# malak29/video-text-detection-system

Hardware: AMD Instinct MI355X
Metric: frames/sec (detect+recognize) @720p, 1/2/4/8 MI355X; box IoU vs CPU ref (higher is better)
Workload: dtype f16

## Files before the change

video-text-detection-system_amd/build_native.py:

```python
import glob
import os
import subprocess
import sys

HERE = os.path.dirname(os.path.abspath(__file__))
CSRC = os.path.join(HERE, "csrc")
OUT_DIR = os.path.join(HERE, "vtd_amd", "_lib")
VARIANT = os.environ.get("VTD_LIB_VARIANT", "")
EXTRA = os.environ.get("VTD_EXTRA_HIPCC_FLAGS", "").split()
if EXTRA and not VARIANT:
    raise SystemExit("VTD_EXTRA_HIPCC_FLAGS needs VTD_LIB_VARIANT=<tag>: the product library is only ever built with the default flags")
OUT = os.path.join(OUT_DIR, f"libvtd_hip_{VARIANT}.so" if VARIANT else "libvtd_hip.so")
OBJ_DIR = os.path.join(HERE, f"build_{VARIANT}" if VARIANT else "build")

COMMON = ["--offload-arch=gfx950", "-O3", "-fPIC", "-std=c++17", "-Wall", "-Wno-unused-function", "-mllvm", "-amdgpu-mfma-vgpr-form",
          "-I" + CSRC] + EXTRA
PER_FILE = {"postprocess.hip": ["-ffp-contract=off"], "adamw.hip": ["-ffp-contract=off"]}


def sources():
    src = glob.glob(os.path.join(CSRC, "*.hip")) + glob.glob(os.path.join(CSRC, "*.cpp"))
    if "-DVTD_EXPERIMENTAL_CANDIDATES" in EXTRA:
        src += glob.glob(os.path.join(CSRC, "experimental", "*.hip"))
    return sorted(src)


def build(force=False, verbose=False):
    os.makedirs(OUT_DIR, exist_ok=True)
    os.makedirs(OBJ_DIR, exist_ok=True)
    headers = (glob.glob(os.path.join(CSRC, "*.h")) + glob.glob(os.path.join(CSRC, "*.inc")) +
               glob.glob(os.path.join(HERE, "..", "include", "*.h")))
    newest_hdr = max(os.path.getmtime(h) for h in headers)
# ... 44 lines not shown
```

video-text-detection-system_amd/csrc/conv_halo.hip:

```cpp
#include <cstdio>
#include <cstdlib>
#include "vtd_common.h"

namespace {

struct HaloParams {
    const half_t* in;
    const half_t* wgt;
    const float* bias;
    const half_t* res;
    half_t* out;
    int n, h, w, cin, cout;
    int in_hp, in_wp, in_ring, out_hp, out_wp, out_ring, res_hp, res_wp, res_ring;
    int tiles_x, tiles_y, tiles_n, relu;
    unsigned long long* stamps;
    int dbg;
};

template <int N>
__device__ __forceinline__ void hl_wait_vmcnt() {
    asm volatile("s_waitcnt vmcnt(%0)" ::"n"(N) : "memory");
}

template <int BN, int TW>
__global__ __launch_bounds__((BN / 64) * 256) void conv_halo_kernel(const HaloParams p) {
    constexpr int WN = BN / 64, NW = 4 * WN, NT = NW * 64, TH = 256 / TW;
    constexpr int HWD = TW + 2, HROWS = (TH + 2) * HWD, HPIECES = (HROWS + 7) / 8, HBYTES = HPIECES * 1024;
    constexpr int HPW = (HPIECES + NW - 1) / NW;
    constexpr int HPS = (HPW + 7) / 8;
    constexpr int BSTAGE = BN * 128, BPW = BN / 8 / NW;
    constexpr int EPI_ROW = BN * 4 + 16;
// ... 499 lines not shown
template <int TW, bool RELU, bool RES>
__global__ __launch_bounds__(512, 1) void conv3x3_c64_duo_kernel(const HaloParams p) {
    constexpr int TH = 256 / TW, HWD = TW + 2, HROWS = (TH + 2) * HWD, HPIECES = (HROWS + 7) / 8, HBYTES = HPIECES * 1024;
    constexpr int HPW = (HPIECES + 3) / 4;
    constexpr int WBYTES = 9 * 64 * 128;
    extern __shared__ __attribute__((aligned(16))) char smem[];
    char* const wl = smem;
    char* const hbuf = smem + WBYTES;

    const int tid = threadIdx.x, lane = tid & 63;
    const int wv = __builtin_amdgcn_readfirstlane(tid >> 6);
    const int g = wv >> 2, w = wv & 3;
    const int lrow = lane >> 3, fr = lane & 15, fq = lane >> 4;
    const int tiles_per_img = p.tiles_x * p.tiles_y, total = p.n * tiles_per_img;

#pragma unroll
    for (int k = 0; k < 9; ++k) {
        const int piece = wv + 8 * k, tap = piece >> 3, row = (piece & 7) * 8 + lrow;
        const int c_log = (lane & 7) ^ ((row >> 1) & 7);
        const int cout = 16 * ((row & 15) >> 2) + 4 * (row >> 4) + (row & 3);
        __builtin_amdgcn_global_load_lds((const VTD_AS1 void*)(p.wgt + cout * 576 + tap * 64 + c_log * 8),
                                         (VTD_AS3 void*)(wl + piece * 1024), 16, 0, 0);
    }
    float* const bias_lds = (float*)(smem + WBYTES + 2 * HBYTES + 1024);
    if (tid < 64) bias_lds[tid] = p.bias[tid];

    auto tile_coords = [&](int t, int& img, int& y0, int& x0) {
        img = t / tiles_per_img;
        const int r = t - img * tiles_per_img, ty = r / p.tiles_x;
        y0 = ty * TH;
        x0 = (r - ty * p.tiles_x) * TW;
    };
    auto issue_halo = [&](int t) {
        int img, y0, x0;
        tile_coords(t, img, y0, x0);
        const half_t* base = p.in + ((int64_t)(img * p.in_hp + y0 - 1 + p.in_ring) * p.in_wp + x0 - 1 + p.in_ring) * 64;
#pragma unroll
        for (int k = 0; k < HPW; ++k) {
            const int piece = w + 4 * k;
            int row = piece * 8 + lrow;
            row = row < HROWS ? row : HROWS - 1;
            const int hy = row / HWD, hx = row - hy * HWD;
            const int hrel = (hy * p.in_wp + hx) * 64 + ((lane & 7) ^ (hx & 6)) * 8;
            const int hdst = piece < HPIECES ? WBYTES + g * HBYTES + piece * 1024 : WBYTES + 2 * HBYTES;
            __builtin_amdgcn_global_load_lds((const VTD_AS1 void*)(base + hrel), (VTD_AS3 void*)(smem + hdst), 16, 0, 0);
        }
    };
    auto px_row = [&](int j) { return (w * 64 + j * 16 + fr) / TW; };
    auto px_col = [&](int j) { return (w * 64 + j * 16 + fr) % TW; };
    const int a_lane_off = (px_row(0) * HWD + px_col(0)) * 128;
    const int b_lane_off = fr * 128;
    const int bswz = (fr >> 1) & 7;
    const char* const hb = hbuf + g * HBYTES;

    const int nq = (total - (int)blockIdx.x + (int)gridDim.x - 1) / (int)gridDim.x;
    const int nmine = (nq - g + 1) >> 1;
    const int phases = 2 * ((nq + 1) >> 1) > 2 * (nq >> 1) + 1 ? 2 * ((nq + 1) >> 1) : 2 * (nq >> 1) + 1;
#ifdef VTD_CONV_EXPERIMENT
    auto block_of = [&](int i) { return p.dbg == 1 ? (int)blockIdx.x : (int)blockIdx.x + (2 * i + g) * (int)gridDim.x; };
#else
    auto block_of = [&](int i) { return (int)blockIdx.x + (2 * i + g) * (int)gridDim.x; };
#endif

    if (nmine > 0) issue_halo(block_of(0));
    hl_wait_vmcnt<0>();
    asm volatile("s_waitcnt lgkmcnt(0)" ::: "memory");
    __builtin_amdgcn_s_barrier();

    floatx4 acc[4][4];
    half8 rv[4][2];
    for (int phase = 0; phase < phases; ++phase) {
        if ((phase & 1) == g) {
            const int i = (phase - g) >> 1;
            if (i < nmine) {
                if (RES) {
                    int img, y0, x0;
                    tile_coords(block_of(i), img, y0, x0);
                    const half_t* rbase = p.res + ((int64_t)(img * p.res_hp + y0 + p.res_ring) * p.res_wp + x0 + p.res_ring) * 64;
#pragma unroll
                    for (int j = 0; j < 4; ++j) {
                        const int rrel = (px_row(j) * p.res_wp + px_col(j)) * 64 + fq * 16;
                        rv[j][0] = *(const half8*)(rbase + rrel);
                        rv[j][1] = *(const half8*)(rbase + rrel + 8);
                    }
                }
#pragma unroll
                for (int a = 0; a < 4; ++a)
#pragma unroll
                    for (int j = 0; j < 4; ++j) acc[a][j] = *(const floatx4*)(bias_lds + fq * 16 + a * 4);
                auto load_frags = [&](int hs, half8 (&af)[4], half8 (&bf)[4]) {
                    const int tap = hs >> 1, kk = hs & 1;
                    const int tapoff = (tap / 3) * HWD + (tap % 3), dx = tap % 3;
// ... 14 lines not shown
#pragma unroll
                        for (int j = 0; j < 4; ++j)
                            acc[a][j] = __builtin_amdgcn_mfma_f32_16x16x32_f16(fb[hs & 1][a], fa[hs & 1][j], acc[a][j], 0, 0, 0);
                    if (hs + 1 < 18) {
                        __builtin_amdgcn_sched_group_barrier(0x100, 8, 0);
                        __builtin_amdgcn_sched_group_barrier(0x008, 16, 0);
                    }
                    __builtin_amdgcn_sched_barrier(0);
                    if (hs + 1 < 18) {
#pragma unroll
                        for (int j = 0; j < 4; ++j) asm volatile("" ::"v"(fa[(hs + 1) & 1][j]));
#pragma unroll
                        for (int a = 0; a < 4; ++a) asm volatile("" ::"v"(fb[(hs + 1) & 1][a]));
                    }
                }
            }
        } else {
            const int i = (phase - g - 1) >> 1;
            if (phase - g - 1 >= 0 && i < nmine) {
                if (i + 1 < nmine) issue_halo(block_of(i + 1));
                int img, y0, x0;
                tile_coords(block_of(i), img, y0, x0);
                half_t* obase = p.out + ((int64_t)(img * p.out_hp + y0 + p.out_ring) * p.out_wp + x0 + p.out_ring) * 64;
#pragma unroll
                for (int j = 0; j < 4; ++j)
#pragma unroll
                    for (int h = 0; h < 2; ++h) {
                        half8 hv;
#pragma unroll
                        for (int k = 0; k < 8; ++k) {
                            float v = acc[2 * h + (k >> 2)][j][k & 3];
                            if (RES) v += (float)rv[j][h][k];
                            hv[k] = (half_t)(RELU ? fmaxf(v, 0.f) : v);
                        }
                        *(half8*)(obase + (px_row(j) * p.out_wp + px_col(j)) * 64 + fq * 16 + h * 8) = hv;
                    }
            }
            hl_wait_vmcnt<0>();
        }
        __builtin_amdgcn_s_barrier();
    }
    hl_wait_vmcnt<0>();
}

template <int TW, bool RELU, bool RES>
int c64_launch(const HaloParams& p, hipStream_t stream) {
    constexpr int TH = 256 / TW, HROWS = (TH + 2) * (TW + 2), HBYTES = (HROWS + 7) / 8 * 1024;
    constexpr int lds = 9 * 64 * 128 + 2 * HBYTES + 1024 + 256;
    static_assert(lds <= 160 * 1024, "LDS budget");
    if (p.h % TH || p.w % TW) return -2205;
    static bool attr_done = false;
    if (!attr_done) {
        hipError_t e = hipFuncSetAttribute((const void*)conv3x3_c64_persistent_kernel<TW, RELU, RES>,
                                           hipFuncAttributeMaxDynamicSharedMemorySize, lds);
        if (e != hipSuccess) return -(int)e;
        attr_done = true;
    }
    const int total = p.n * p.tiles_y * p.tiles_x;
    const int grid = total < 256 ? total : 256;
    static const bool want_stamps = [] { const char* e = getenv("VTD_HALO_STAMPS"); return e && e[0] == '1'; }();
    if (want_stamps) {
        HaloParams q = p;
        unsigned long long* dev = nullptr;
// ... 2 lines not shown
        hipLaunchKernelGGL((conv3x3_c64_persistent_kernel<TW, RELU, RES>), dim3(grid), dim3(256), lds, stream, q);
        (void)hipStreamSynchronize(stream);
        unsigned long long* h = (unsigned long long*)malloc((size_t)grid * 32);
        (void)hipMemcpy(h, dev, (size_t)grid * 32, hipMemcpyDeviceToHost);
        double a = 0, b = 0, c = 0;
        for (int i = 0; i < grid; ++i) { a += (double)h[4 * i + 1]; b += (double)(h[4 * i + 2] - h[4 * i + 1]); c += (double)(h[4 * i + 3] - h[4 * i + 2]); }
        const double blocks = (double)total / grid;
        fprintf(stderr, "[c64 stamps] res=%d blocks/WG %.1f: per block ticks: issue+wait %.1f  K-loop %.1f  epilogue %.1f\n", (int)RES, blocks,
                a / grid / blocks, b / grid / blocks, c / grid / blocks);
        free(h);
        (void)hipFree(dev);
        return 0;
    }
    const char* duo_env = getenv("VTD_C64_DUO");
    const bool duo = !(duo_env && duo_env[0] == '0');
#ifdef VTD_CONV_EXPERIMENT
    if (duo) {
        HaloParams q = p;
        const char* d = getenv("VTD_C64_DEBUG");
        q.dbg = d ? atoi(d) : 0;
        hipError_t e = hipFuncSetAttribute((const void*)conv3x3_c64_duo_kernel<TW, RELU, RES>, hipFuncAttributeMaxDynamicSharedMemorySize, lds);
        if (e != hipSuccess) return -(int)e;
        hipLaunchKernelGGL((conv3x3_c64_duo_kernel<TW, RELU, RES>), dim3(grid), dim3(512), lds, stream, q);
        return -(int)hipGetLastError();
    }
#endif
    if (duo) {
        static bool attr_duo = false;
        if (!attr_duo) {
            hipError_t e = hipFuncSetAttribute((const void*)conv3x3_c64_duo_kernel<TW, RELU, RES>, hipFuncAttributeMaxDynamicSharedMemorySize, lds);
            if (e != hipSuccess) return -(int)e;
            attr_duo = true;
        }
        hipLaunchKernelGGL((conv3x3_c64_duo_kernel<TW, RELU, RES>), dim3(grid), dim3(512), lds, stream, p);
        return -(int)hipGetLastError();
    }
    hipLaunchKernelGGL((conv3x3_c64_persistent_kernel<TW, RELU, RES>), dim3(grid), dim3(256), lds, stream, p);
    return -(int)hipGetLastError();
}

template <int TW>
int c64_dispatch(const HaloParams& p, hipStream_t stream) {
    if (p.relu) return p.res ? c64_launch<TW, true, true>(p, stream) : c64_launch<TW, true, false>(p, stream);
    return p.res ? c64_launch<TW, false, true>(p, stream) : c64_launch<TW, false, false>(p, stream);
}

template <int BN, int TW>
int halo_launch(const HaloParams& p, hipStream_t stream) {
    constexpr int TH = 256 / TW, HROWS = (TH + 2) * (TW + 2), HBYTES = (HROWS + 7) / 8 * 1024;
// ... 46 lines not shown
    if (c.in_y0 < 0 || c.in_x0 != c.in_y0 || c.ho <= 0 || c.wo <= 0 || c.M % (c.ho * c.wo)) return false;
    const int h = c.ho, w = c.wo;
    auto eff = [&](int th, int tw) { return (double)h * w / ((double)((h + th - 1) / th * th) * ((w + tw - 1) / tw * tw)); };
    const double e16 = eff(16, 16), e32 = eff(8, 32);
    const int tw = e16 >= e32 ? 16 : 32;
    if ((tw == 16 ? e16 : e32) < 0.85) return false;
    *tw_out = tw;
    *bn_out = (c.cout % 128 == 0) ? 128 : 64;
    return true;
}

bool vtd_conv_halo_c64_supported(const ConvParams& c, int tw) {
    return c.in_c == 64 && c.cout == 64 && c.wo % tw == 0 && c.ho % (256 / tw) == 0;
}

int vtd_launch_conv_halo(const ConvParams& c, int bn, int tw, hipStream_t stream) {
    HaloParams p;
    p.in = c.in; p.wgt = c.wgt; p.bias = c.bias; p.res = (c.flags & EPI_RESIDUAL) ? c.res : nullptr; p.out = (half_t*)c.out;
    p.h = c.ho; p.w = c.wo; p.n = c.M / (c.ho * c.wo); p.cin = c.in_c; p.cout = c.cout;
    p.in_hp = c.in_hp; p.in_wp = c.in_wp; p.in_ring = c.in_y0 + 1;
    p.out_hp = c.out_hp; p.out_wp = c.out_wp; p.out_ring = c.out_ring;
    p.res_hp = c.res_hp; p.res_wp = c.res_wp; p.res_ring = c.res_ring;
    p.relu = (c.flags & EPI_RELU) ? 1 : 0;
    p.stamps = nullptr;
    p.dbg = 0;
    if (c.in_y0 != c.in_x0 || c.in_y0 < 0 || c.K != 9 * c.in_c || c.out_c != c.cout || p.n <= 0 || (c.in_c & 63) || (c.cout & 63) ||
        (tw != 16 && tw != 32) || c.stride != 1 || c.M != p.n * c.ho * c.wo)
        return -2201;
    if ((int64_t)p.n * c.in_hp * c.in_wp * c.in_c >= (1ll << 31)) return -2202;
    const int th = 256 / tw;
    p.tiles_x = (p.w + tw - 1) / tw; p.tiles_y = (p.h + th - 1) / th; p.tiles_n = bn > 1 ? p.cout / bn : 1;
    if (bn == 2) {
// ... 15 lines not shown
```

video-text-detection-system_amd/csrc/stem_pool.hip:

```cpp
#include <cstdlib>
#include "vtd_common.h"

namespace {

constexpr int SP_PT_ROWS = 7, SP_PT_COLS = 8;
constexpr int SP_CT_COLS = 17;
constexpr int SP_PATCH_COLS = 40;
constexpr int SP_PIECES = 12;
constexpr int SP_PATCH_BYTES = SP_PIECES * 1024;
constexpr int SP_NST = 3;
constexpr int SP_CT_PITCH = 144;
constexpr int SP_LDS = SP_NST * SP_PATCH_BYTES + 256 * SP_CT_PITCH + 256;

struct StemPoolParams {
    const half_t* in;
    const half_t* w;
    const float* bias;
    half_t* out;
    int n, in_hp, in_wp, conv_h, conv_w, pool_h, pool_w, out_hp, out_wp, out_ring;
    int tiles_x, tiles_y, total_tiles;
};

typedef short short4v __attribute__((ext_vector_type(4)));
typedef short short8v __attribute__((ext_vector_type(8)));
__device__ __forceinline__ half8 sp_max(half8 a, half8 b) {
    return __builtin_bit_cast(half8, __builtin_elementwise_max(__builtin_bit_cast(short8v, a), __builtin_bit_cast(short8v, b)));
}

__host__ __device__ constexpr int sp_chan(int tile, int row) { return 32 * (tile >> 1) + 8 * (row >> 2) + 4 * (tile & 1) + (row & 3); }

template <int N>
__device__ __forceinline__ void sp_wait_vmcnt() { asm volatile("s_waitcnt vmcnt(%0)" ::"n"(N) : "memory"); }
__device__ __forceinline__ void sp_lds_barrier() {
    asm volatile("s_waitcnt lgkmcnt(0)" ::: "memory");
    __builtin_amdgcn_s_barrier();
// ... 6 lines not shown
    const int ty = r / p.tiles_x;
    py0 = ty * SP_PT_ROWS;
    px0 = (r - ty * p.tiles_x) * SP_PT_COLS;
}

template <int DBG>
__global__ __launch_bounds__(256, 2) void stem_pool_kernel(const StemPoolParams p) {
    extern __shared__ __attribute__((aligned(16))) unsigned char sp_smem[];
    unsigned char* const ring = sp_smem;
    unsigned char* const ctile = sp_smem + SP_NST * SP_PATCH_BYTES;
    float* const bias_lds = (float*)(ctile + 256 * SP_CT_PITCH);
    const int tid = threadIdx.x, lane = tid & 63;
    const int wv = __builtin_amdgcn_readfirstlane(tid >> 6);
    const int fr = lane & 15, fq = lane >> 4;

    int first, stride, last;
    if ((gridDim.x & 7) == 0) {
        const int xcd = blockIdx.x & 7, per = gridDim.x >> 3;
        const int lo = (int)(((int64_t)p.total_tiles * xcd) >> 3);
        last = (int)(((int64_t)p.total_tiles * (xcd + 1)) >> 3);
        first = lo + (blockIdx.x >> 3);
        stride = per;
    } else {
        first = blockIdx.x; stride = gridDim.x; last = p.total_tiles;
    }
    if (first >= last) return;
    const int nt = (last - first + stride - 1) / stride;

    half8 wreg[7][4];
#pragma unroll
    for (int ky = 0; ky < 7; ++ky)
#pragma unroll
        for (int i = 0; i < 4; ++i) wreg[ky][i] = *(const half8*)(p.w + ((ky * 4 + i) * 64 + lane) * 8);
    if (tid < 64) bias_lds[tid] = p.bias[tid];
    int a_off[4];
#pragma unroll
    for (int j = 0; j < 4; ++j) {
        const int pix = wv * 64 + j * 16 + fr;
        const int c_row = pix / SP_CT_COLS, c_col = pix - c_row * SP_CT_COLS;
        a_off[j] = ((2 * c_row) * SP_PATCH_COLS + 2 * c_col + 2 * fq) * 8;
    }
    int u_row[3], u_col[3];
// ... 10 lines not shown
        sp_tile_coords(p, __builtin_amdgcn_readfirstlane(tile), img, py0, px0);
        const half_t* base = p.in + (int64_t)img * p.in_hp * p.in_wp * 4;
#pragma unroll
        for (int k = 0; k < 3; ++k) {
            int iy = 4 * py0 - 2 + u_row[k], ix = 4 * px0 - 2 + u_col[k];
            iy = iy < 0 ? 0 : iy > p.in_hp - 1 ? p.in_hp - 1 : iy;
            ix = ix < 0 ? 0 : ix > p.in_wp - 2 ? p.in_wp - 2 : ix;
            __builtin_amdgcn_global_load_lds((const VTD_AS1 void*)(base + (iy * p.in_wp + ix) * 4),
                                             (VTD_AS3 void*)(ring + stage * SP_PATCH_BYTES + (wv + 4 * k) * 1024), 16, 0, 0);
        }
    };

    if constexpr (DBG == 7 || DBG == 8) {
        if (((blockIdx.x >> 3) & 32) != 0) { __builtin_amdgcn_s_sleep(60); }
    }
    issue(first, 0);
    if (nt > 1) { issue(first + stride, 1); sp_wait_vmcnt<3>(); } else sp_wait_vmcnt<0>();
    sp_lds_barrier();

    int st = 0;
    for (int k = 0; k < nt; ++k) {
        const int tile = first + k * stride;
        int img, py0, px0;
        sp_tile_coords(p, __builtin_amdgcn_readfirstlane(tile), img, py0, px0);
        if (k + 2 < nt) issue(tile + 2 * stride, st == 0 ? SP_NST - 1 : st - 1);

        floatx4 acc[4][4];
#pragma unroll
        for (int i = 0; i < 4; ++i)
#pragma unroll
            for (int j = 0; j < 4; ++j) acc[i][j] = *(const floatx4*)(bias_lds + sp_chan(i, fq * 4));
        const unsigned char* pb = ring + st * SP_PATCH_BYTES;
        half8 af[2][4];
#pragma unroll
        for (int j = 0; j < 4; ++j) af[0][j] = *(const half8*)(pb + a_off[j]);
        if constexpr (DBG == 6 || DBG == 7) __builtin_amdgcn_s_setprio(3);
#pragma unroll
        for (int ky = 0; ky < 7; ++ky) {
            if (ky < 6) {
#pragma unroll
// ... 2 lines not shown
            if (DBG == 3 && ky > 0) { for (int j = 0; j < 4; ++j) asm volatile("" ::"v"(af[ky & 1][j])); continue; }
#pragma unroll
            for (int j = 0; j < 4; ++j)
#pragma unroll
                for (int i = 0; i < 4; ++i) acc[i][j] = __builtin_amdgcn_mfma_f32_16x16x32_f16(wreg[ky][i], af[ky & 1][j], acc[i][j], 0, 0, 0);
            if (ky < 6) __builtin_amdgcn_sched_group_barrier(0x100, 4, 0);
            __builtin_amdgcn_sched_group_barrier(0x008, 16, 0);
            __builtin_amdgcn_sched_barrier(0);
        }

        if constexpr (DBG == 6 || DBG == 7) __builtin_amdgcn_s_setprio(0);
        if constexpr (DBG == 2) {
            float t = 0.f;
            for (int i = 0; i < 4; ++i) for (int j = 0; j < 4; ++j) t += acc[i][j][0] + acc[i][j][1] + acc[i][j][2] + acc[i][j][3];
            if (t == 123.456f) p.out[0] = (half_t)t;
            if (k + 2 < nt) sp_wait_vmcnt<3>(); else sp_wait_vmcnt<0>();
            sp_lds_barrier();
            st = st + 1 == SP_NST ? 0 : st + 1;
            continue;
        }
#pragma unroll
        for (int j = 0; j < 4; ++j) {
            const int pix = wv * 64 + j * 16 + fr;
            const int c_row = pix / SP_CT_COLS, c_col = pix - c_row * SP_CT_COLS;
            const int cy = 2 * py0 - 1 + c_row, cx = 2 * px0 - 1 + c_col;
            const bool valid = cy >= 0 && cy < p.conv_h && cx >= 0 && cx < p.conv_w;
            unsigned char* dst = ctile + pix * SP_CT_PITCH + fq * 16;
#pragma unroll
            for (int k = 0; k < 2; ++k) {
                typedef float float2v __attribute__((ext_vector_type(2)));
                typedef _Float16 half2v __attribute__((ext_vector_type(2)));
                const floatx4 a = acc[2 * k][j], b = acc[2 * k + 1][j];
                const half2v h0 = __builtin_convertvector((float2v{a[0], a[1]}), half2v);
                const half2v h1 = __builtin_convertvector((float2v{a[2], a[3]}), half2v);
                const half2v h2 = __builtin_convertvector((float2v{b[0], b[1]}), half2v);
                const half2v h3 = __builtin_convertvector((float2v{b[2], b[3]}), half2v);
                half8 hv = half8{h0[0], h0[1], h1[0], h1[1], h2[0], h2[1], h3[0], h3[1]};
                hv = __builtin_bit_cast(half8, __builtin_elementwise_max(__builtin_bit_cast(short8v, hv), short8v{0, 0, 0, 0, 0, 0, 0, 0}));
                if (!valid) hv = half8{0, 0, 0, 0, 0, 0, 0, 0};
                *(half8*)(dst + k * 64) = hv;
            }
        }
        sp_lds_barrier();

        if constexpr (DBG != 1) {
            const int cg = (lane >> 2) & 7;
            const int qx = ((lane >> 5) & 1) | ((lane & 3) << 1);
            const bool two = wv < 3;
            const unsigned char* src0 = ctile + ((2 * wv) * SP_CT_COLS + 2 * qx) * SP_CT_PITCH + cg * 16;
            const int px = px0 + qx;
#pragma unroll
            for (int it = 0; it < 2; ++it) {
                if (it == 1 && !two) break;
                const unsigned char* src = src0 + it * (8 * SP_CT_COLS * SP_CT_PITCH);
                half8 v[9];
#pragma unroll
                for (int r = 0; r < 3; ++r)
#pragma unroll
                    for (int c = 0; c < 3; ++c) v[r * 3 + c] = *(const half8*)(src + (r * SP_CT_COLS + c) * SP_CT_PITCH);
                __builtin_amdgcn_sched_group_barrier(0x100, 9, 0);
                half8 m = sp_max(v[0], v[1]);
#pragma unroll
                for (int q = 2; q < 9; ++q) m = sp_max(m, v[q]);
                const int py = py0 + wv + 4 * it;
                if (DBG == 5) asm volatile("" ::"v"(m));
                else if (py < p.pool_h && px < p.pool_w)
                    *(half8*)(p.out + (((int64_t)img * p.out_hp + py + p.out_ring) * p.out_wp + px + p.out_ring) * 64 + cg * 8) = m;
            }
        }
        if (k + 2 < nt) sp_wait_vmcnt<3>(); else sp_wait_vmcnt<0>();
        sp_lds_barrier();
        st = st + 1 == SP_NST ? 0 : st + 1;
    }
}

}

void vtd_stem_pool_pack_weights(const float* w_folded , half_t* packed ) {
    for (int ky = 0; ky < 7; ++ky)
        for (int i = 0; i < 4; ++i)
            for (int lane = 0; lane < 64; ++lane) {
                const int fr = lane & 15, fq = lane >> 4, co = sp_chan(i, fr);
                for (int e = 0; e < 8; ++e) {
                    const int kx = 2 * fq + (e >> 2), c = e & 3;
                    float v = 0.f;
                    if (kx < 7 && c < 3) v = w_folded[((co * 3 + c) * 7 + ky) * 7 + kx];
                    packed[((ky * 4 + i) * 64 + lane) * 8 + e] = (half_t)v;
                }
            }
}

int vtd_launch_stem_pool(const TensorDesc& in, const TensorDesc& out, const half_t* w_packed, const float* bias, int n,
                         hipStream_t stream) {
    if (in.c != 4 || in.ring != 3 || out.c != 64 || (in.h & 3) || (in.w & 3) || out.h != in.h / 4 || out.w != in.w / 4 ||
        in.hp != in.h + 6 || in.wp != in.w + 6 || (in.wp & 1) || n <= 0 || n > in.n || n > out.n)
        return -2001;
    if (out.w % SP_PT_COLS) return -2002;
    StemPoolParams p;
    p.in = in.ptr; p.w = w_packed; p.bias = bias; p.out = out.ptr;
    p.n = n; p.in_hp = in.hp; p.in_wp = in.wp; p.conv_h = in.h / 2; p.conv_w = in.w / 2; p.pool_h = out.h; p.pool_w = out.w;
    p.out_hp = out.hp; p.out_wp = out.wp; p.out_ring = out.ring;
    p.tiles_x = out.w / SP_PT_COLS;
    p.tiles_y = (out.h + SP_PT_ROWS - 1) / SP_PT_ROWS;
    p.total_tiles = n * p.tiles_x * p.tiles_y;
    const int grid = p.total_tiles < 512 ? p.total_tiles : 512;
    void (*kern)(const StemPoolParams) = stem_pool_kernel<0>;
#ifdef VTD_STEM_EXPERIMENT
    if (const char* e = getenv("VTD_STEM_DEBUG")) {
        switch (atoi(e)) {
            case 1: kern = stem_pool_kernel<1>; break;
            case 2: kern = stem_pool_kernel<2>; break;
            case 3: kern = stem_pool_kernel<3>; break;
            case 4: kern = stem_pool_kernel<4>; break;
            case 5: kern = stem_pool_kernel<5>; break;
            case 6: kern = stem_pool_kernel<6>; break;
            case 7: kern = stem_pool_kernel<7>; break;
            case 8: kern = stem_pool_kernel<8>; break;
            default: break;
        }
    }
// ... 18 lines not shown
```

video-text-detection-system_amd/csrc/vtd_api.cpp:

```cpp
#include <algorithm>
#include <cmath>
#include <cstdio>
#include <cstdlib>
#include <cstring>
#include <map>
#include <memory>
#include <string>
#include <vector>

#include "../../include/vtd.h"
#include "vtd_common.h"

int vtd_launch_conv(const ConvParams& p, int cfg, hipStream_t stream);
int vtd_conv_num_configs();
bool vtd_conv_config_valid(const ConvParams& p, int cfg);
int vtd_launch_preprocess(const uint8_t* frames, int n, int H, int W, half_t* out, const int* xb, const int* xk, int ksx,
                          const int* yb, const int* yk, int ksy, int max_rows, hipStream_t stream);
int vtd_launch_nchw_to_input(const float* x, half_t* out, int n, hipStream_t stream);
int vtd_launch_maxpool(const TensorDesc& in, const TensorDesc& out, int n, int kh, int kw, int sh, int sw, int pad_h, int pad_w,
                       hipStream_t stream);
void vtd_stem_pool_pack_weights(const float* w_folded, half_t* packed);
int vtd_launch_stem_pool(const TensorDesc& in, const TensorDesc& out, const half_t* w_packed, const float* bias, int n, hipStream_t stream);
extern "C" int vtd_head_entry_halo_steps(int py, int px, int nch1, int* out);
int vtd_launch_head_entry_halo(const ConvParams& c, const int* steps_dev, int nsteps, int big_tiles, hipStream_t stream);
#ifdef VTD_EXPERIMENTAL_CANDIDATES
extern "C" int vtd_head_entry_half_schedule(const int* steps, int nsteps, int* out);
int vtd_launch_head_entry_half(const ConvParams& c, const int* sched_dev, int nsteps, hipStream_t stream);
int vtd_head_entry_pair_tables(int py, int px, int c2ch, int* half_steps, int* plan);
int vtd_launch_head_entry_pair(const ConvParams& c, const int* half_steps_dev, const int* plan_dev, int nh, hipStream_t stream);
#endif
bool vtd_conv_halo_supported(const ConvParams& c, int* bn_out, int* tw_out);
bool vtd_conv_halo_c64_supported(const ConvParams& c, int tw);
int vtd_launch_conv_halo(const ConvParams& c, int bn, int tw, hipStream_t stream);
bool vtd_pointwise128_supported(const ConvParams& c);
int vtd_launch_pointwise128(const ConvParams& c, hipStream_t stream);
void vtd_head_tail_pack_w1(const half_t* w1_gemm, half_t* packed);
void vtd_head_tail_pack_w2(const float* w2, half_t* packed);
int vtd_launch_head_tail(const TensorDesc& in, const half_t* w1, const float* bias1, const half_t* w2, float b2, float* out, int n,
                         hipStream_t stream);

int vtd_launch_crop_resize(const uint8_t* frames, int H, int W, const int32_t* boxes, int ncrops, uint8_t* out, hipStream_t s);
int vtd_launch_crnn_conv1(const uint8_t* in_u8, const float* in_f32, const half_t* w, const float* bias, half_t* out, int n, hipStream_t s);
int vtd_launch_lstm(const half_t* xs, const half_t* whh, half_t* hout, int D, int T, hipStream_t s);
int vtd_launch_ctc_greedy(const float* logits, int n, int T, int V, int ld, const int32_t* id2char, int blank, int apply_softmax,
                          int32_t* out, hipStream_t s);
int vtd_launch_compact_rows(const float* in, float* out, int64_t rows, int V, int ld, hipStream_t s);
int vtd_dbloss_ws_bytes();
int vtd_launch_dbloss(const float* prob, const float* thresh, const float* prob_t, const float* thresh_t, int64_t n, float smooth, double* workspace,
// ... 135 lines not shown
    int tiles_border = 0;
    const int* he_steps = nullptr;
    int he_nsteps = 0;
    const int* hh_sched = nullptr;
    const int* hp_half_steps = nullptr;
    const int* hp_plan = nullptr;
    int hp_nh = 0;
    const int* tile_combo_b = nullptr;
    int tiles_per_img_b = 0;
    int tiles_per_img = 0, seg1_steps = 0, cin_steps2 = 0, kw2 = 0, s_step2 = 0, r_step2 = 0, img_h = 0, img_w = 0;
    TensorDesc in2;
    const float* bias_tab = nullptr;
    bool dual = false;
    int in2_mul = 1, in2_shr = 0;
    int pool_pw = 0;
};

struct Op {
    enum Kind { CONV, POOL, FINAL, STEMPOOL, HEADTAIL, BORDER } kind;
    ConvOp conv;
    TensorDesc pin, pout;
    int pk[6] = {0, 0, 0, 0, 0, 0};
    const float* fw = nullptr;
    float fbias = 0.f;
    int final_slot = 0;
    const half_t* spw = nullptr;
    const float* spb = nullptr;
    const half_t* htw1 = nullptr;
    const half_t* htw2 = nullptr;
};

static void fill_conv_params(const ConvOp& c, int n, ConvParams& p) {
    std::memset(&p, 0, sizeof(p));
    p.in = c.in.ptr; p.wgt = c.w; p.k_hi_step = c.k_hi_step; p.cin_steps = c.cin_steps; p.kw = c.kw; p.s_step = c.s_step; p.r_step = c.r_step; p.bias = c.bias;
    p.res = c.has_res ? c.res.ptr : nullptr;
    p.out = (c.flags & (EPI_OUT_F32 | EPI_OUT_F16)) ? c.out_f32 : (void*)c.out.ptr;
    p.M = n * c.ho * c.wo; p.K = c.K; p.cout = c.cout; p.cout_pad = c.cout_pad;
    p.ho = c.ho; p.wo = c.wo;
    p.in_hp = c.in.hp; p.in_wp = c.in.wp; p.in_c = c.in.c; p.in_y0 = c.in_y0; p.in_x0 = c.in_x0; p.stride = c.stride;
    p.out_hp = c.out.hp; p.out_wp = c.out.wp; p.out_c = c.out.c; p.out_ring = c.out.ring;
    p.res_hp = c.res.hp; p.res_wp = c.res.wp; p.res_ring = c.res.ring; p.res_shift = c.res_shift;
    p.ps_cout = c.ps_cout; p.flags = c.flags; p.ldc = c.ldc;
    p.seg_cols = c.seg_cols;
    for (int i = 0; i < 3; ++i) { p.seg_out[i] = c.seg_out[i]; p.seg_ldc[i] = c.seg_ldc[i]; }
// ... 66 lines not shown
    }
    if (cfg == kHeadEntryHalfCfg) {
        if (!c.hh_sched || !c.tile_combo_border) return ERR_GEOMETRY;
        return vtd_launch_head_entry_half(p, c.hh_sched, c.he_nsteps, s);
    }
#else
    if (cfg == kHeadEntryPairCfg || cfg == kHeadEntryHalfCfg) return ERR_GEOMETRY;
#endif
    if (cfg == kHeadEntryHaloCfg || cfg == kHeadEntryHalo256Cfg) {
        if (!c.he_steps || !c.tile_combo_border) return ERR_GEOMETRY;
        return vtd_launch_head_entry_halo(p, c.he_steps, c.he_nsteps, cfg == kHeadEntryHalo256Cfg ? 1 : 0, s);
    }
    if (cfg == kHaloCfg || cfg == kHaloC64Cfg || cfg == kHalo64Cfg) {
        int bn = 0, tw = 0;
        if (!vtd_conv_halo_supported(p, &bn, &tw)) return ERR_GEOMETRY;
        return vtd_launch_conv_halo(p, cfg == kHaloC64Cfg ? 1 : cfg == kHalo64Cfg ? 2 : bn, tw, s);
    }
    if (cfg == kPointwiseCfg) return vtd_launch_pointwise128(p, s);
    if (!c.plist && (cfg == 0 || cfg == 12 || cfg == 13 || cfg == 14 || cfg == 15)) cfg = pick_tile_height(p, cfg);
    return vtd_launch_conv(p, cfg, s);
}

static int launch_border_tiles(const ConvOp& c, int n, hipStream_t s) {
    if (!c.tile_combo_border || c.tiles_border <= 0) return ERR_GEOMETRY;
    ConvParams pb;
    fill_conv_params(c, n, pb);
    pb.tile_combo = c.tile_combo_border; pb.tiles_per_img = c.tiles_border; pb.M = n * c.tiles_border * 128;
    pb.plist_b = nullptr; pb.tile_combo_b = nullptr; pb.tiles_per_img_b = 0;
    return vtd_launch_conv(pb, 9, s);
}

// ... 1319 lines not shown
    if (!known_detector_key(k)) return ERR_UNKNOWN_KEY;
    if (k.size() > 19 && k.compare(k.size() - 19, 19, "num_batches_tracked") == 0) return 0;
    d->sd[k].assign(host_data, host_data + numel);
    return 0;
}

int vtd_detector_set_option(vtd_detector* d, const char* name, int value) {
    if (!d || !name || d->finalized) return ERR_ARG;
    if (std::string(name) == "fuse_fpn_head") { d->fuse_fpn_head = value != 0; return 0; }
    if (std::string(name) == "fuse_stem_pool") { d->fuse_stem_pool = value != 0; return 0; }
    if (std::string(name) == "head_tail_kernel") { d->head_tail_kernel = value != 0; return 0; }
    if (std::string(name) == "fuse_downsample") { d->fuse_downsample = value != 0; return 0; }
    return ERR_UNKNOWN_KEY;
}

int vtd_detector_finalize(vtd_detector* d, vtd_stream stream) {
    if (!d) return ERR_ARG;
    if (d->finalized) return ERR_ARG;
    int rc = build_detector_graph(d);
    if (rc) return rc;
    hipError_t e = hipStreamSynchronize((hipStream_t)stream);
    if (e != hipSuccess) return -(int)e;
    d->sd.clear();
    d->finalized = true;
    return 0;
}

int vtd_detector_preprocess(vtd_detector* d, const uint8_t* frames_dev, int n, int height, int width, vtd_stream stream) {
    if (!d || !frames_dev || height <= 0 || width <= 0) return ERR_ARG;
    if (!d->finalized) return ERR_NOT_FINALIZED;
    if (n <= 0 || n > d->max_batch) return ERR_BATCH;
    PreTables t;
    int rc = get_pre_tables(d, height, width, t);
    if (rc) return rc;
    return vtd_launch_preprocess(frames_dev, n, height, width, d->input.ptr, t.xb, t.xk, t.ksx, t.yb, t.yk, t.ksy, t.max_rows,
// ... 31 lines not shown
        const bool prof = d->profiling && (d->prof_only < 0 || d->prof_only == (int)oi);
        if (prof) {
            e0 = d->take_event();
            e1 = d->take_event();
            if (!e0 || !e1) return ERR_ARG;
            VTD_HIP_CHECK(hipEventRecord(e0, s));
        }
        switch (o.kind) {
            case Op::CONV: rc = launch_conv_op(o.conv, n, s, cfgs[oi]); break;
            case Op::POOL: rc = vtd_launch_maxpool(o.pin, o.pout, n, o.pk[0], o.pk[1], o.pk[2], o.pk[3], o.pk[4], o.pk[5], s); break;
            case Op::FINAL: rc = launch_conv_op(o.conv, n, s, 7, outs[o.final_slot]); break;
            case Op::HEADTAIL:
                rc = vtd_launch_head_tail(o.conv.in, o.htw1, o.conv.bias, o.htw2, o.conv.head_b, outs[o.final_slot], n, s);
                break;
            case Op::BORDER: rc = launch_border_tiles(o.conv, n, s); break;
            case Op::STEMPOOL: rc = vtd_launch_stem_pool(o.pin, o.pout, o.spw, o.spb, n, s); break;
        }
        if (rc) return rc;
        if (prof) {
            VTD_HIP_CHECK(hipEventRecord(e1, s));
            d->ev_spans.push_back({(int)oi, {e0, e1}});
            d->prof_macs[oi] += (o.kind != Op::POOL) ? (double)o.conv.macs_per_image * n : 0.0;
        }
    }
    return 0;
}

int vtd_detector_forward(vtd_detector* d, int n, float* prob_dev, float* thresh_dev, vtd_stream stream) {
    if (!d || !prob_dev) return ERR_ARG;
    if (!d->finalized) return ERR_NOT_FINALIZED;
    if (n <= 0 || n > d->max_batch) return ERR_BATCH;
// ... 402 lines not shown
```

video-text-detection-system_amd/csrc/vtd_common.h:

```cpp
#pragma once
#include <hip/hip_runtime.h>
#include <stdint.h>

typedef _Float16 half_t;
typedef half_t half8 __attribute__((ext_vector_type(8)));
typedef half_t half4 __attribute__((ext_vector_type(4)));
typedef half_t half2v __attribute__((ext_vector_type(2)));
typedef float floatx4 __attribute__((ext_vector_type(4)));

#define VTD_AS1 __attribute__((address_space(1)))
#define VTD_AS3 __attribute__((address_space(3)))

struct TensorDesc {
    half_t* ptr;
    int n, h, w, c;
    int ring;
    int hp, wp;
};

static inline __host__ __device__ int64_t tensor_elems(const TensorDesc& t) {
    return (int64_t)t.n * t.hp * t.wp * t.c;
}

enum : int {
// ... 41 lines not shown
    const int* tile_combo_b;
    int tiles_per_img_b;
    int tiles_per_img;
    const half_t* in2;
    int in2_hp, in2_wp, in2_c, in2_ring;
    int in2_mul, in2_shr;
    int seg1_steps;
    int cin_steps2, kw2, s_step2, r_step2;
    const float* bias_tab;
    int img_h, img_w;
    const float* head_w;
    float head_b;
    float* prob_out;
};

#define VTD_HIP_CHECK(expr)                                   \
    do {                                                      \
        hipError_t _e = (expr);                               \
        if (_e != hipSuccess) return -(int)_e;                \
    } while (0)
```

Baseline: 12040.

## Add per-XCD dynamic tile claiming via atomic counters to c64 conv and stem-pool

Replaces the static round-robin tile assignment in the 64-channel 3x3 duo conv kernel and the stem+pool kernel with work stealing from per-XCD global atomic counters. Each block draws its next tile while computing the current one. The last block to retire resets the counters for the next launch. The aim is to even out load imbalance and tail effects across CUs and XCDs. The cost is extra atomics and LDS handoffs per tile, and tiles may lose locality. The atomic optimizer is disabled for these files, and an env var turns the feature off.

```diff
diff --git a/video-text-detection-system_amd/build_native.py b/video-text-detection-system_amd/build_native.py
--- a/video-text-detection-system_amd/build_native.py
+++ b/video-text-detection-system_amd/build_native.py
@@ -16,6 +16,8 @@
 COMMON = ["--offload-arch=gfx950", "-O3", "-fPIC", "-std=c++17", "-Wall", "-Wno-unused-function", "-mllvm", "-amdgpu-mfma-vgpr-form",
           "-I" + CSRC] + EXTRA
 PER_FILE = {"postprocess.hip": ["-ffp-contract=off"], "adamw.hip": ["-ffp-contract=off"]}
+for _f in ("conv_halo.hip", "stem_pool.hip"):
+    PER_FILE[_f] = ["-mllvm", "-amdgpu-atomic-optimizer-strategy=None"]
 
 
 def sources():
diff --git a/video-text-detection-system_amd/csrc/conv_halo.hip b/video-text-detection-system_amd/csrc/conv_halo.hip
--- a/video-text-detection-system_amd/csrc/conv_halo.hip
+++ b/video-text-detection-system_amd/csrc/conv_halo.hip
@@ -15,6 +15,7 @@
     int tiles_x, tiles_y, tiles_n, relu;
     unsigned long long* stamps;
     int dbg;
+    int* claim;
 };
 
 template <int N>
@@ -544,6 +545,31 @@
     const int lrow = lane >> 3, fr = lane & 15, fq = lane >> 4;
     const int tiles_per_img = p.tiles_x * p.tiles_y, total = p.n * tiles_per_img;
 
+    float* const bias_lds = (float*)(smem + WBYTES + 2 * HBYTES + 1024);
+    VTD_AS3 int* const claim_lds = (VTD_AS3 int*)(bias_lds + 64);
+    const bool claimer = (wv & 3) == 0 && lane == 0;
+    int* const counter = p.claim + (blockIdx.x & 7) * VTD_CLAIM_STRIDE;
+    auto draw = [&]() { return __hip_atomic_fetch_add(counter, 1, __ATOMIC_RELAXED, __HIP_MEMORY_SCOPE_AGENT); };
+    auto resolve = [&](int got) { const int t = 8 * got + (int)(blockIdx.x & 7); return got >= 0 && t < total ? t : -1; };
+    auto static_block = [&](int k) { const int t = (int)blockIdx.x + (2 * k + g) * (int)gridDim.x; return t < total ? t : -1; };
+    if (claimer) {
+        int b = static_block(0);
+        if (p.claim) b = resolve(draw());
+        claim_lds[g] = b;
+    }
+    __syncthreads();
+    int mine0 = __builtin_amdgcn_readfirstlane(claim_lds[0]), mine1 = __builtin_amdgcn_readfirstlane(claim_lds[1]);
+    auto retire = [&]() {
+        if (p.claim && tid == 0 &&
+            __hip_atomic_fetch_add(p.claim + 8 * VTD_CLAIM_STRIDE, 1, __ATOMIC_RELAXED, __HIP_MEMORY_SCOPE_AGENT) == (int)gridDim.x - 1) {
+            for (int i = 0; i < 9; ++i) __hip_atomic_store(p.claim + i * VTD_CLAIM_STRIDE, 0, __ATOMIC_RELAXED, __HIP_MEMORY_SCOPE_AGENT);
+        }
+    };
+    if (mine0 < 0 && mine1 < 0) {
+        retire();
+        return;
+    }
+
 #pragma unroll
     for (int k = 0; k < 9; ++k) {
         const int piece = wv + 8 * k, tap = piece >> 3, row = (piece & 7) * 8 + lrow;
@@ -552,10 +578,12 @@
         __builtin_amdgcn_global_load_lds((const VTD_AS1 void*)(p.wgt + cout * 576 + tap * 64 + c_log * 8),
                                          (VTD_AS3 void*)(wl + piece * 1024), 16, 0, 0);
     }
-    float* const bias_lds = (float*)(smem + WBYTES + 2 * HBYTES + 1024);
     if (tid < 64) bias_lds[tid] = p.bias[tid];
 
     auto tile_coords = [&](int t, int& img, int& y0, int& x0) {
+#ifdef VTD_CONV_EXPERIMENT
+        if (p.dbg == 1) t = (int)blockIdx.x;
+#endif
         img = t / tiles_per_img;
         const int r = t - img * tiles_per_img, ty = r / p.tiles_x;
         y0 = ty * TH;
@@ -583,29 +611,28 @@
     const int bswz = (fr >> 1) & 7;
     const char* const hb = hbuf + g * HBYTES;
 
-    const int nq = (total - (int)blockIdx.x + (int)gridDim.x - 1) / (int)gridDim.x;
-    const int nmine = (nq - g + 1) >> 1;
-    const int phases = 2 * ((nq + 1) >> 1) > 2 * (nq >> 1) + 1 ? 2 * ((nq + 1) >> 1) : 2 * (nq >> 1) + 1;
-#ifdef VTD_CONV_EXPERIMENT
-    auto block_of = [&](int i) { return p.dbg == 1 ? (int)blockIdx.x : (int)blockIdx.x + (2 * i + g) * (int)gridDim.x; };
-#else
-    auto block_of = [&](int i) { return (int)blockIdx.x + (2 * i + g) * (int)gridDim.x; };
-#endif
-
-    if (nmine > 0) issue_halo(block_of(0));
+    if ((g ? mine1 : mine0) >= 0) issue_halo(g ? mine1 : mine0);
     hl_wait_vmcnt<0>();
     asm volatile("s_waitcnt lgkmcnt(0)" ::: "memory");
     __builtin_amdgcn_s_barrier();
 
+    int pend0 = -1, pend1 = -1;
+    int nclaimed = 1;
     floatx4 acc[4][4];
     half8 rv[4][2];
-    for (int phase = 0; phase < phases; ++phase) {
-        if ((phase & 1) == g) {
-            const int i = (phase - g) >> 1;
-            if (i < nmine) {
+    for (int phase = 0; mine0 >= 0 || mine1 >= 0 || pend0 >= 0 || pend1 >= 0; ++phase) {
+        const int c = phase & 1;
+        const int claimed = __builtin_amdgcn_readfirstlane(claim_lds[c ^ 1]);
+        const int s_pend = c ? pend0 : pend1;
+        const int s_next = s_pend >= 0 ? claimed : -1;
+        const int c_mine = c ? mine1 : mine0;
+        if (c == g) {
+            if (c_mine >= 0) {
+                int got = -1;
+                if (claimer && p.claim) got = draw();
                 if (RES) {
                     int img, y0, x0;
-                    tile_coords(block_of(i), img, y0, x0);
+                    tile_coords(c_mine, img, y0, x0);
                     const half_t* rbase = p.res + ((int64_t)(img * p.res_hp + y0 + p.res_ring) * p.res_wp + x0 + p.res_ring) * 64;
 #pragma unroll
                     for (int j = 0; j < 4; ++j) {
@@ -650,13 +677,15 @@
                         for (int a = 0; a < 4; ++a) asm volatile("" ::"v"(fb[(hs + 1) & 1][a]));
                     }
                 }
+                if (claimer) claim_lds[g] = p.claim ? resolve(got) : static_block(nclaimed);
+                ++nclaimed;
+                asm volatile("s_waitcnt lgkmcnt(0)" ::: "memory");
             }
         } else {
-            const int i = (phase - g - 1) >> 1;
-            if (phase - g - 1 >= 0 && i < nmine) {
-                if (i + 1 < nmine) issue_halo(block_of(i + 1));
+            if (s_pend >= 0) {
+                if (s_next >= 0) issue_halo(s_next);
                 int img, y0, x0;
-                tile_coords(block_of(i), img, y0, x0);
+                tile_coords(s_pend, img, y0, x0);
                 half_t* obase = p.out + ((int64_t)(img * p.out_hp + y0 + p.out_ring) * p.out_wp + x0 + p.out_ring) * 64;
 #pragma unroll
                 for (int j = 0; j < 4; ++j)
@@ -675,14 +704,22 @@
             hl_wait_vmcnt<0>();
         }
         __builtin_amdgcn_s_barrier();
+        if (c) {
+            pend1 = mine1; mine1 = -1;
+            if (pend0 >= 0) { mine0 = s_next; pend0 = -1; }
+        } else {
+            pend0 = mine0; mine0 = -1;
+            if (pend1 >= 0) { mine1 = s_next; pend1 = -1; }
+        }
     }
     hl_wait_vmcnt<0>();
+    retire();
 }
 
 template <int TW, bool RELU, bool RES>
 int c64_launch(const HaloParams& p, hipStream_t stream) {
     constexpr int TH = 256 / TW, HROWS = (TH + 2) * (TW + 2), HBYTES = (HROWS + 7) / 8 * 1024;
-    constexpr int lds = 9 * 64 * 128 + 2 * HBYTES + 1024 + 256;
+    constexpr int lds = 9 * 64 * 128 + 2 * HBYTES + 1024 + 256 + 64;
     static_assert(lds <= 160 * 1024, "LDS budget");
     if (p.h % TH || p.w % TW) return -2205;
     static bool attr_done = false;
@@ -715,9 +752,12 @@
     }
     const char* duo_env = getenv("VTD_C64_DUO");
     const bool duo = !(duo_env && duo_env[0] == '0');
+    const char* claim_env = getenv("VTD_TILE_CLAIM");
+    HaloParams pc = p;
+    if (claim_env && claim_env[0] == '0') pc.claim = nullptr;
 #ifdef VTD_CONV_EXPERIMENT
     if (duo) {
-        HaloParams q = p;
+        HaloParams q = pc;
         const char* d = getenv("VTD_C64_DEBUG");
         q.dbg = d ? atoi(d) : 0;
         hipError_t e = hipFuncSetAttribute((const void*)conv3x3_c64_duo_kernel<TW, RELU, RES>, hipFuncAttributeMaxDynamicSharedMemorySize, lds);
@@ -733,7 +773,7 @@
             if (e != hipSuccess) return -(int)e;
             attr_duo = true;
         }
-        hipLaunchKernelGGL((conv3x3_c64_duo_kernel<TW, RELU, RES>), dim3(grid), dim3(512), lds, stream, p);
+        hipLaunchKernelGGL((conv3x3_c64_duo_kernel<TW, RELU, RES>), dim3(grid), dim3(512), lds, stream, pc);
         return -(int)hipGetLastError();
     }
     hipLaunchKernelGGL((conv3x3_c64_persistent_kernel<TW, RELU, RES>), dim3(grid), dim3(256), lds, stream, p);
@@ -810,8 +850,9 @@
     return c.in_c == 64 && c.cout == 64 && c.wo % tw == 0 && c.ho % (256 / tw) == 0;
 }
 
-int vtd_launch_conv_halo(const ConvParams& c, int bn, int tw, hipStream_t stream) {
+int vtd_launch_conv_halo(const ConvParams& c, int bn, int tw, hipStream_t stream, int* claim) {
     HaloParams p;
+    p.claim = bn == 1 ? claim : nullptr;
     p.in = c.in; p.wgt = c.wgt; p.bias = c.bias; p.res = (c.flags & EPI_RESIDUAL) ? c.res : nullptr; p.out = (half_t*)c.out;
     p.h = c.ho; p.w = c.wo; p.n = c.M / (c.ho * c.wo); p.cin = c.in_c; p.cout = c.cout;
     p.in_hp = c.in_hp; p.in_wp = c.in_wp; p.in_ring = c.in_y0 + 1;
diff --git a/video-text-detection-system_amd/csrc/stem_pool.hip b/video-text-detection-system_amd/csrc/stem_pool.hip
--- a/video-text-detection-system_amd/csrc/stem_pool.hip
+++ b/video-text-detection-system_amd/csrc/stem_pool.hip
@@ -10,7 +10,7 @@
 constexpr int SP_PATCH_BYTES = SP_PIECES * 1024;
 constexpr int SP_NST = 3;
 constexpr int SP_CT_PITCH = 144;
-constexpr int SP_LDS = SP_NST * SP_PATCH_BYTES + 256 * SP_CT_PITCH + 256;
+constexpr int SP_LDS = SP_NST * SP_PATCH_BYTES + 256 * SP_CT_PITCH + 256 + 16;
 
 struct StemPoolParams {
     const half_t* in;
@@ -19,6 +19,7 @@
     half_t* out;
     int n, in_hp, in_wp, conv_h, conv_w, pool_h, pool_w, out_hp, out_wp, out_ring;
     int tiles_x, tiles_y, total_tiles;
+    int* claim;
 };
 
 typedef short short4v __attribute__((ext_vector_type(4)));
@@ -55,18 +56,48 @@
     const int wv = __builtin_amdgcn_readfirstlane(tid >> 6);
     const int fr = lane & 15, fq = lane >> 4;
 
+    const bool dyn = DBG == 0 && p.claim != nullptr && (gridDim.x & 7) == 0;
+    auto eighth_lo = [&](int x) { return (int)(((int64_t)p.total_tiles * x) >> 3); };
     int first, stride, last;
     if ((gridDim.x & 7) == 0) {
         const int xcd = blockIdx.x & 7, per = gridDim.x >> 3;
-        const int lo = (int)(((int64_t)p.total_tiles * xcd) >> 3);
-        last = (int)(((int64_t)p.total_tiles * (xcd + 1)) >> 3);
-        first = lo + (blockIdx.x >> 3);
+        last = eighth_lo(xcd + 1);
+        first = eighth_lo(xcd) + (blockIdx.x >> 3);
         stride = per;
     } else {
         first = blockIdx.x; stride = gridDim.x; last = p.total_tiles;
     }
-    if (first >= last) return;
-    const int nt = (last - first + stride - 1) / stride;
+    auto static_tile = [&](int k) { const int t = first + k * stride; return t < last ? t : -1; };
+    int* const counter = p.claim + (blockIdx.x & 7) * VTD_CLAIM_STRIDE;
+    const int my_lo = eighth_lo(blockIdx.x & 7), my_hi = eighth_lo((blockIdx.x & 7) + 1);
+    auto draw = [&](int count) { return __hip_atomic_fetch_add(counter, count, __ATOMIC_RELAXED, __HIP_MEMORY_SCOPE_AGENT); };
+    auto resolve = [&](int got) { const int t = my_lo + got; return got >= 0 && t < my_hi ? t : -1; };
+    auto retire = [&]() {
+        if (dyn && tid == 0 &&
+            __hip_atomic_fetch_add(p.claim + 8 * VTD_CLAIM_STRIDE, 1, __ATOMIC_RELAXED, __HIP_MEMORY_SCOPE_AGENT) == (int)gridDim.x - 1) {
+            for (int i = 0; i < 9; ++i) __hip_atomic_store(p.claim + i * VTD_CLAIM_STRIDE, 0, __ATOMIC_RELAXED, __HIP_MEMORY_SCOPE_AGENT);
+        }
+    };
+    VTD_AS3 int* const tile_lds = (VTD_AS3 int*)(bias_lds + 64);
+    int t0, t1, t2;
+    if (dyn) {
+        if (tid == 0) {
+            const int g0 = draw(3);
+            tile_lds[0] = resolve(g0);
+            tile_lds[1] = resolve(g0 + 1);
+            tile_lds[2] = resolve(g0 + 2);
+        }
+        __syncthreads();
+        t0 = __builtin_amdgcn_readfirstlane(tile_lds[0]);
+        t1 = __builtin_amdgcn_readfirstlane(tile_lds[1]);
+        t2 = __builtin_amdgcn_readfirstlane(tile_lds[2]);
+    } else {
+        t0 = static_tile(0); t1 = static_tile(1); t2 = static_tile(2);
+    }
+    if (t0 < 0) {
+        retire();
+        return;
+    }
 
     half8 wreg[7][4];
 #pragma unroll
@@ -107,16 +138,19 @@
     if constexpr (DBG == 7 || DBG == 8) {
         if (((blockIdx.x >> 3) & 32) != 0) { __builtin_amdgcn_s_sleep(60); }
     }
-    issue(first, 0);
-    if (nt > 1) { issue(first + stride, 1); sp_wait_vmcnt<3>(); } else sp_wait_vmcnt<0>();
+    issue(t0, 0);
+    if (t1 >= 0) { issue(t1, 1); sp_wait_vmcnt<3>(); } else sp_wait_vmcnt<0>();
     sp_lds_barrier();
 
     int st = 0;
-    for (int k = 0; k < nt; ++k) {
-        const int tile = first + k * stride;
+    for (int k = 0; t0 >= 0; ++k, t0 = t1, t1 = t2) {
+        if (k > 0) t2 = dyn ? __builtin_amdgcn_readfirstlane(tile_lds[0]) : static_tile(k + 2);
+        int got = -1;
+        if (dyn && tid == 0 && t2 >= 0) got = draw(1);
+        const int tile = t0;
         int img, py0, px0;
         sp_tile_coords(p, __builtin_amdgcn_readfirstlane(tile), img, py0, px0);
-        if (k + 2 < nt) issue(tile + 2 * stride, st == 0 ? SP_NST - 1 : st - 1);
+        if (t2 >= 0) issue(t2, st == 0 ? SP_NST - 1 : st - 1);
 
         floatx4 acc[4][4];
 #pragma unroll
@@ -149,7 +183,7 @@
             float t = 0.f;
             for (int i = 0; i < 4; ++i) for (int j = 0; j < 4; ++j) t += acc[i][j][0] + acc[i][j][1] + acc[i][j][2] + acc[i][j][3];
             if (t == 123.456f) p.out[0] = (half_t)t;
-            if (k + 2 < nt) sp_wait_vmcnt<3>(); else sp_wait_vmcnt<0>();
+            if (t2 >= 0) sp_wait_vmcnt<3>(); else sp_wait_vmcnt<0>();
             sp_lds_barrier();
             st = st + 1 == SP_NST ? 0 : st + 1;
             continue;
@@ -177,6 +211,7 @@
             }
         }
         sp_lds_barrier();
+        if (dyn && tid == 0) tile_lds[0] = resolve(got);
 
         if constexpr (DBG != 1) {
             const int cg = (lane >> 2) & 7;
@@ -203,10 +238,11 @@
                     *(half8*)(p.out + (((int64_t)img * p.out_hp + py + p.out_ring) * p.out_wp + px + p.out_ring) * 64 + cg * 8) = m;
             }
         }
-        if (k + 2 < nt) sp_wait_vmcnt<3>(); else sp_wait_vmcnt<0>();
+        if (t2 >= 0) sp_wait_vmcnt<3>(); else sp_wait_vmcnt<0>();
         sp_lds_barrier();
         st = st + 1 == SP_NST ? 0 : st + 1;
     }
+    retire();
 }
 
 }
@@ -226,7 +262,7 @@
 }
 
 int vtd_launch_stem_pool(const TensorDesc& in, const TensorDesc& out, const half_t* w_packed, const float* bias, int n,
-                         hipStream_t stream) {
+                         hipStream_t stream, int* claim) {
     if (in.c != 4 || in.ring != 3 || out.c != 64 || (in.h & 3) || (in.w & 3) || out.h != in.h / 4 || out.w != in.w / 4 ||
         in.hp != in.h + 6 || in.wp != in.w + 6 || (in.wp & 1) || n <= 0 || n > in.n || n > out.n)
         return -2001;
@@ -238,7 +274,10 @@
     p.tiles_x = out.w / SP_PT_COLS;
     p.tiles_y = (out.h + SP_PT_ROWS - 1) / SP_PT_ROWS;
     p.total_tiles = n * p.tiles_x * p.tiles_y;
-    const int grid = p.total_tiles < 512 ? p.total_tiles : 512;
+    const char* claim_env = getenv("VTD_TILE_CLAIM");
+    p.claim = (claim_env && claim_env[0] == '0') ? nullptr : claim;
+    int grid = p.total_tiles < 512 ? p.total_tiles : 512;
+    if (p.claim && grid < 512) grid = (grid + 7) & ~7;
     void (*kern)(const StemPoolParams) = stem_pool_kernel<0>;
 #ifdef VTD_STEM_EXPERIMENT
     if (const char* e = getenv("VTD_STEM_DEBUG")) {
diff --git a/video-text-detection-system_amd/csrc/vtd_api.cpp b/video-text-detection-system_amd/csrc/vtd_api.cpp
--- a/video-text-detection-system_amd/csrc/vtd_api.cpp
+++ b/video-text-detection-system_amd/csrc/vtd_api.cpp
@@ -20,7 +20,8 @@
 int vtd_launch_maxpool(const TensorDesc& in, const TensorDesc& out, int n, int kh, int kw, int sh, int sw, int pad_h, int pad_w,
                        hipStream_t stream);
 void vtd_stem_pool_pack_weights(const float* w_folded, half_t* packed);
-int vtd_launch_stem_pool(const TensorDesc& in, const TensorDesc& out, const half_t* w_packed, const float* bias, int n, hipStream_t stream);
+int vtd_launch_stem_pool(const TensorDesc& in, const TensorDesc& out, const half_t* w_packed, const float* bias, int n, hipStream_t stream,
+                         int* claim = nullptr);
 extern "C" int vtd_head_entry_halo_steps(int py, int px, int nch1, int* out);
 int vtd_launch_head_entry_halo(const ConvParams& c, const int* steps_dev, int nsteps, int big_tiles, hipStream_t stream);
 #ifdef VTD_EXPERIMENTAL_CANDIDATES
@@ -31,7 +32,7 @@
 #endif
 bool vtd_conv_halo_supported(const ConvParams& c, int* bn_out, int* tw_out);
 bool vtd_conv_halo_c64_supported(const ConvParams& c, int tw);
-int vtd_launch_conv_halo(const ConvParams& c, int bn, int tw, hipStream_t stream);
+int vtd_launch_conv_halo(const ConvParams& c, int bn, int tw, hipStream_t stream, int* claim = nullptr);
 bool vtd_pointwise128_supported(const ConvParams& c);
 int vtd_launch_pointwise128(const ConvParams& c, hipStream_t stream);
 void vtd_head_tail_pack_w1(const half_t* w1_gemm, half_t* packed);
@@ -197,6 +198,7 @@
     bool dual = false;
     int in2_mul = 1, in2_shr = 0;
     int pool_pw = 0;
+    int* claim = nullptr;
 };
 
 struct Op {
@@ -211,6 +213,7 @@
     const float* spb = nullptr;
     const half_t* htw1 = nullptr;
     const half_t* htw2 = nullptr;
+    int* claim = nullptr;
 };
 
 static void fill_conv_params(const ConvOp& c, int n, ConvParams& p) {
@@ -307,7 +310,7 @@
     if (cfg == kHaloCfg || cfg == kHaloC64Cfg || cfg == kHalo64Cfg) {
         int bn = 0, tw = 0;
         if (!vtd_conv_halo_supported(p, &bn, &tw)) return ERR_GEOMETRY;
-        return vtd_launch_conv_halo(p, cfg == kHaloC64Cfg ? 1 : cfg == kHalo64Cfg ? 2 : bn, tw, s);
+        return vtd_launch_conv_halo(p, cfg == kHaloC64Cfg ? 1 : cfg == kHalo64Cfg ? 2 : bn, tw, s, c.claim);
     }
     if (cfg == kPointwiseCfg) return vtd_launch_pointwise128(p, s);
     if (!c.plist && (cfg == 0 || cfg == 12 || cfg == 13 || cfg == 14 || cfg == 15)) cfg = pick_tile_height(p, cfg);
@@ -1657,11 +1660,26 @@
     return ERR_UNKNOWN_KEY;
 }
 
+static int alloc_claim_words(vtd_detector* d) {
+    void* base = nullptr;
+    int rc = d->arena.alloc(&base, d->ops.size() * VTD_CLAIM_BYTES, true);
+    if (rc) return rc;
+    for (size_t oi = 0; oi < d->ops.size(); ++oi) {
+        Op& o = d->ops[oi];
+        int* words = (int*)((char*)base + oi * VTD_CLAIM_BYTES);
+        if (o.kind == Op::STEMPOOL) o.claim = words;
+        const ConvOp& c = o.conv;
+        if (o.kind == Op::CONV && !c.plist && !c.dual && c.in.c == 64 && c.cout == 64 && c.K == 9 * 64 && c.stride == 1) o.conv.claim = words;
+    }
+    return 0;
+}
+
 int vtd_detector_finalize(vtd_detector* d, vtd_stream stream) {
     if (!d) return ERR_ARG;
     if (d->finalized) return ERR_ARG;
     int rc = build_detector_graph(d);
     if (rc) return rc;
+    if ((rc = alloc_claim_words(d))) return rc;
     hipError_t e = hipStreamSynchronize((hipStream_t)stream);
     if (e != hipSuccess) return -(int)e;
     d->sd.clear();
@@ -1723,7 +1741,7 @@
                 rc = vtd_launch_head_tail(o.conv.in, o.htw1, o.conv.bias, o.htw2, o.conv.head_b, outs[o.final_slot], n, s);
                 break;
             case Op::BORDER: rc = launch_border_tiles(o.conv, n, s); break;
-            case Op::STEMPOOL: rc = vtd_launch_stem_pool(o.pin, o.pout, o.spw, o.spb, n, s); break;
+            case Op::STEMPOOL: rc = vtd_launch_stem_pool(o.pin, o.pout, o.spw, o.spb, n, s, o.claim); break;
         }
         if (rc) return rc;
         if (prof) {
diff --git a/video-text-detection-system_amd/csrc/vtd_common.h b/video-text-detection-system_amd/csrc/vtd_common.h
--- a/video-text-detection-system_amd/csrc/vtd_common.h
+++ b/video-text-detection-system_amd/csrc/vtd_common.h
@@ -79,6 +79,9 @@
     float* prob_out;
 };
 
+constexpr int VTD_CLAIM_STRIDE = 64;
+constexpr int VTD_CLAIM_BYTES = 9 * VTD_CLAIM_STRIDE * 4;
+
 #define VTD_HIP_CHECK(expr)                                   \
     do {                                                      \
         hipError_t _e = (expr);                               \
```

New measurement: 11930. About the same (-0.9%).
